# ginolhac/mapDamage

Measured on AMD Instinct MI355X. Metric: reads/sec (misincorporation+comp tables), higher is better.
Workload: dtype u8

## Files before the change

### include/mdx.h

```cpp
#ifndef MDX_H
#define MDX_H

#include <stdint.h>

#ifdef __cplusplus
extern "C" {
#endif

#define MDX_ABI_VERSION 6

#define MDX_OK 0
#define MDX_ERR_ARG (-1)
#define MDX_ERR_HIP (-2)
#define MDX_ERR_STATE (-3)
#define MDX_ERR_MASK_INDEX (-4)
#define MDX_ERR_LGD_OVERFLOW (-5)
#define MDX_ERR_BAD_READ (-6)

#define MDX_ERR_UNSUPPORTED (-8)
#define MDX_ERR_COMM (-7)

#define MDX_FLAG_QUAL_ABOVE_MIN 0x8000
#define MDX_FLAG_HAS_QUAL 0x4000

// ... 145 lines not shown
                       uint8_t *d_qual_out, double *d_mr_raw, uint8_t *d_status);
int mdx_tabulate_rescale_device(mdx_ctx *ctx, const mdx_batch *dev_batch, const int32_t *d_mtid, const int32_t *d_mpos,
                                uint8_t *d_qual_out, double *d_mr_raw, uint8_t *d_status);
int mdx_rescale_patches_device(mdx_ctx *ctx, const mdx_batch *dev_batch, const int32_t *d_mtid, const int32_t *d_mpos,
                               uint64_t *d_patch, int64_t patch_cap, int32_t n_parts, uint64_t *d_n_patch, double *d_mr_raw,
                               uint8_t *d_status);
int mdx_tabulate_rescale_patches_device(mdx_ctx *ctx, const mdx_batch *dev_batch, const int32_t *d_mtid, const int32_t *d_mpos,
                                        uint64_t *d_patch, int64_t patch_cap, int32_t n_parts, uint64_t *d_n_patch, double *d_mr_raw,
                                        uint8_t *d_status);
int mdx_rescale_expand_device(mdx_ctx *ctx, const mdx_batch *dev_batch, const uint64_t *d_patch, int64_t patch_cap, int32_t n_parts,
                              const uint64_t *d_n_patch, uint8_t *d_qual_out);
int mdx_rescale_timing_read(mdx_ctx *ctx, int64_t *n_launches, double *total_ms);
int64_t mdx_fused_launches(const mdx_ctx *ctx);
int64_t mdx_packed_launches(const mdx_ctx *ctx);
int64_t mdx_geo_spec_launches(const mdx_ctx *ctx);
int64_t mdx_libsorts(const mdx_ctx *ctx);
int mdx_last_launch_geometry(const mdx_ctx *ctx, int32_t out[4]);
int64_t mdx_rescale_summary_words(const mdx_ctx *ctx);
int mdx_rescale_summary(mdx_ctx *ctx, uint64_t *words);

typedef struct mdx_source mdx_source;
int mdx_source_open(const char *path, mdx_source **out);
const char *mdx_source_error(const mdx_source *source);
int mdx_source_is_stream(const mdx_source *source);
int mdx_source_peek(mdx_source *source, uint8_t *buf, int32_t n, int32_t *got);
int64_t mdx_source_read(mdx_source *source, uint8_t *buf, int64_t cap);
int mdx_source_seek(mdx_source *source, int64_t offset);
void mdx_source_close(mdx_source *source);

typedef struct mdx_bam mdx_bam;
// ... 141 lines not shown
```

### mapdamage_amd/build.py

```python

import os
import pathlib
import shutil
import subprocess

HERE = pathlib.Path(__file__).resolve().parent
CSRC = HERE / "csrc"
LIB = HERE / "libmdx.so"
SOURCES = ["mdx_kernels.hip", "mdx_rescale.hip", "mdx_capi.cpp", "mdx_bamio.cpp", "mdx_gbam.hip", "mdx_samio.cpp", "mdx_gsam.hip", "mdx_libsort.hip", "mdx_strata.hip", "mdx_fasta.hip", "mdx_stats.hip", "mdx_dedup.hip", "mdx_depth.hip", "mdx_pileup.hip"]
HEADERS = [CSRC / "mdx_internal.h", CSRC / "mdx_filter.h", CSRC / "mdx_damage_key.h", CSRC / "mdx_pmd_key.h", CSRC / "mdx_dup_key.h", CSRC / "mdx_dup_table.h", CSRC / "mdx_depth_key.h", CSRC / "mdx_pileup_key.h", CSRC / "mdx_kept.h", CSRC / "mdx_kept_tags.h", CSRC / "mdx_kept_index.h", CSRC / "mdx_kept_mask.h", CSRC / "mdx_kept_md.h", CSRC / "mdx_device.h", CSRC / "mdx_inflate.h", CSRC / "mdx_deflate.h", CSRC / "mdx_crc32.h", HERE.parent / "include" / "mdx.h"]


def hipcc():
    exe = shutil.which("hipcc") or "/opt/rocm/bin/hipcc"
    if not os.path.exists(exe):
        raise RuntimeError("hipcc not found; the HIP extension cannot be built")
    return exe


def needs_build():
    if not LIB.exists():
        return True
    t = LIB.stat().st_mtime
    deps = [CSRC / s for s in SOURCES] + HEADERS
    return any(p.stat().st_mtime > t for p in deps)
# ... 51 lines not shown
```

### mapdamage_amd/csrc/mdx_capi.cpp

```cpp
#include "../../include/mdx.h"
#include "mdx_internal.h"

#include <dlfcn.h>

#include <chrono>

#include <cstdio>
#include <cstdlib>
#include <cstring>
#include <mutex>
#include <new>
#include <string>
#include <thread>
#include <utility>
#include <vector>

namespace {

constexpr size_t kLdsLimit = MDX_LDS_LIMIT;
#ifdef MDX_WAVE_CLK
static unsigned long long *g_dbg_clk = nullptr;
extern "C" int mdx_dbg_clk_read(unsigned long long *out, int n) {
    if (!g_dbg_clk) return -1;
    (void)hipDeviceSynchronize();
// ... 102 lines not shown
    int st_turn = 0;
    void *gbam_arena = nullptr;
    size_t gbam_arena_cap = 0;
    void *gbam_tables = nullptr;
    void *gbam_stream = nullptr, *gbam_event = nullptr;
    int64_t record_base = 0;
    DevBuf unpacked;
    DevBuf lists;
    DevBuf rs_part;
    DevBuf rs_lists;
    DevBuf rs_in;
    uint32_t *d_tile_ctr = nullptr;
    size_t fuse_prepared = 0;
    size_t pkf_prepared = 0;
    MdxPkConfig pk = {512, 0};
    bool tile_ctr_clean = false;
    bool pkm_prepared = false;
    DevBuf lowq;
    DevBuf libsort;
    DevBuf libsort_scratch;
    const void *libsort_checked = nullptr;
    uint64_t libsort_checked_sig = 0;
    DevBuf ml_partials;
    struct Strata {
        StrataKind kind = STRATA_NONE;
        int n_groups = 0;
        unsigned long long *d_strata_kept = nullptr;
        int32_t *d_group_of_tid = nullptr;
        int strata_n_contig = 0;
        void *d_regions = nullptr;
        MdxRegions regions = {};
// ... 95 lines not shown
    } while (0)

#define HIP_TRY(ctx, call)                                                                     \
    do {                                                                                       \
        hipError_t e_ = (call);                                                                \
        if (e_ != hipSuccess)                                                                  \
            return fail((ctx), MDX_ERR_HIP, std::string(#call) + ": " + hipGetErrorString(e_)); \
    } while (0)

int64_t lgd_words(const mdx_ctx *c) { return (int64_t)c->cfg.nlib * 4 * c->cfg.lgd_max; }
int64_t mis_words(const mdx_ctx *c) { return (int64_t)c->cfg.nlib * 4 * c->cfg.length * MDX_N_MIS_COLS; }
int64_t comp_words(const mdx_ctx *c) { return (int64_t)c->cfg.nlib * 4 * (c->cfg.length + c->cfg.around) * 4; }

size_t pmd_hist_words(const mdx_ctx *c) { return (size_t)(c->cfg.nlib / (c->strata.pmd_n_thresholds + 1)) * MDX_PMD_BINS + 1; }

int zero_accumulators(mdx_ctx *c) {
    HIP_TRY(c, hipMemsetAsync(c->d_raw, 0, (size_t)c->dims.w_total * 8, c->stream));
    HIP_TRY(c, hipMemsetAsync(c->d_lgd_dense, 0, (size_t)lgd_words(c) * 8 * c->lgd_copies, c->stream));
    HIP_TRY(c, hipMemsetAsync(c->d_n_lgd_over, 0, 8, c->stream));
    HIP_TRY(c, hipMemsetAsync(c->d_err, 0xFF, 8, c->stream));
    if (c->strata.d_strata_kept) HIP_TRY(c, hipMemsetAsync(c->strata.d_strata_kept, 0, (size_t)c->cfg.nlib * 8, c->stream));
    if (c->strata.d_pmd_hist) HIP_TRY(c, hipMemsetAsync(c->strata.d_pmd_hist, 0, pmd_hist_words(c) * 8, c->stream));
    return MDX_OK;
}

template <class Key>
Key key_args(const mdx_ctx *c, const mdx_batch *b) {
    Key k{};
    k.n = b->n_reads; k.n_cigar = b->n_cigar; k.n_bases = b->n_bases;
    k.flag = b->flag; k.lib = b->lib; k.tid = b->tid; k.pos = b->pos;
    k.cigar_off = b->cigar_off; k.cigar = b->cigar; k.seq_off = b->seq_off; k.seq = b->seq;
// ... 156 lines not shown
        delete c;
        return MDX_ERR_HIP;
    }
    *out = c;
    if (cfg->nlib > 65535)
        return fail(c, MDX_ERR_ARG, "more than 65535 tables (libraries x reference groups): the 16-bit library column names "
                                    "no more, 0xFFFF being the record without a library");
    HIP_TRY(c, hipSetDevice(cfg->device));
    hipDeviceProp_t prop;
    HIP_TRY(c, hipGetDeviceProperties(&prop, cfg->device));
    c->n_cu = prop.multiProcessorCount > 0 ? prop.multiProcessorCount : 256;
    if (const char *e = getenv("MDX_TEST_CUS")) {
        const int n = atoi(e);
        if (n >= 1 && n < c->n_cu) c->n_cu = n;
    }
    HIP_TRY(c, hipStreamCreateWithFlags(&c->own_stream, hipStreamNonBlocking));
    c->stream = c->own_stream;
    lap("context, stream");

    const int lgd_lds = mdx_k_lgd_lds(cfg->length, cfg->around, cfg->lgd_max);
    if ((int64_t)cfg->nlib * (4LL * cfg->length * 29 + 8LL * (2LL * cfg->around + 512) +
                              4LL * lgd_lds + 128) > 0x7FFFFFF0LL || cfg->length > (1 << 24) || cfg->around > (1 << 24))
        return fail(c, MDX_ERR_ARG, "table too large (nlib * length)");
    c->dims = mdx_make_dims(cfg->length, cfg->around, cfg->nlib, cfg->lgd_max, lgd_lds);
    int group = cfg->nlib;
    while (group > 1 && mdx_k_lds_bytes(mdx_make_dims(cfg->length, cfg->around, group, cfg->lgd_max, lgd_lds)) > kLdsLimit)
        group--;
    const MdxDims gdims = mdx_make_dims(cfg->length, cfg->around, group, cfg->lgd_max, lgd_lds);
    c->lds_bytes = mdx_k_lds_bytes(gdims);
    if (c->lds_bytes <= kLdsLimit) {
        c->mode = MDX_MODE_LDS;
        c->lib_group = group;
        c->max_grid = c->n_cu * (2048 / mdx_k_block_threads());
        HIP_TRY(c, mdx_k_prepare(c->lds_bytes));
        {
            const MdxDims d1 = mdx_make_dims(cfg->length, cfg->around, 1, cfg->lgd_max, lgd_lds);
            c->pk = mdx_k_pk_config(d1, kLdsLimit);
            HIP_TRY(c, mdx_k_prepare_packed(mdx_k_pk_lds_bytes(d1, c->pk)));
            if (const char *e = getenv("MDX_DEBUG_PK")) if (*e && *e != '0')
                fprintf(stderr, "[mdx] packed kernels: blocks of %d threads, %zu bytes of LDS, columns %s\n", c->pk.threads, mdx_k_pk_lds_bytes(d1, c->pk),
                        c->pk.pfl ? "prefetched into the LDS" : "by plain loads");
        }
        lap("kernels");
        HIP_TRY(c, hipMalloc((void **)&c->d_partials, (size_t)c->max_grid * gdims.w_total * 4));
    } else {
        c->mode = MDX_MODE_GLOBAL;
        c->max_grid = c->n_cu * (2048 / mdx_k_block_threads());
    }
    HIP_TRY(c, hipMalloc((void **)&c->d_raw, (size_t)c->dims.w_total * 8));
    c->lgd_copies = mdx_lgd_copies_for(cfg->nlib, cfg->lgd_max);
    HIP_TRY(c, hipMalloc((void **)&c->d_lgd_dense, (size_t)lgd_words(c) * 8 * c->lgd_copies));
    HIP_TRY(c, hipMalloc((void **)&c->d_lgd_over, (size_t)(cfg->lgd_over_cap > 0 ? cfg->lgd_over_cap : 1) * 32));
    HIP_TRY(c, hipMalloc((void **)&c->d_n_lgd_over, 8));
    HIP_TRY(c, hipMalloc((void **)&c->d_err, 8));
    int rc = zero_accumulators(c);
    if (rc != MDX_OK) return rc;
    HIP_TRY(c, hipStreamSynchronize(c->stream));
    lap("accumulators");
    return MDX_OK;
// ... 477 lines not shown
            const int64_t n_tiles = (b->n_reads + T - 1) / T;
            const int64_t n_pools = mdx_n_pools((unsigned)grid);
            const int64_t chunk = MDX_POOL_CHUNK;
            const int64_t pool_tiles = ((n_tiles + n_pools * chunk - 1) / (n_pools * chunk)) * chunk, pool_waves = (grid / n_pools) * wpb_l;
            const bool quota = fuse || (pmask && !ml);
            a.tile_quota = quota ? (int)(2 * ((pool_tiles + pool_waves - 1) / pool_waves) + 2) : 0x7FFFFFFF;
            a.list_cap = fuse ? (int64_t)a.tile_quota * T + 128 : 0;
            a.round_tiles = MDX_ROUND_TILES;
            a.ring_size = MDX_LIST_RING;
            if (quota) while ((int64_t)a.ring_size < (int64_t)a.tile_quota * T + 128) a.ring_size *= 2;
            if (!c->d_tile_ctr) {
                HIP_TRY(c, hipMalloc((void **)&c->d_tile_ctr, (size_t)MDX_CTR_WORDS * 4));
                HIP_TRY(c, hipMemsetAsync(c->d_tile_ctr, 0, (size_t)MDX_CTR_WORDS * 4, c->stream));
            }
            if (n_pools * MDX_CTR_PAD > MDX_CTR_WORDS / 2 || n_pools * MDX_CTR_PAD > MDX_CTR_WORDS) return fail(c, MDX_ERR_STATE, "more blocks than tile counters");
            a.tile_ctr = c->d_tile_ctr;
            {
                const size_t list_bytes = (size_t)nwaves * (size_t)MDX_WAVE_SCRATCH(a.ring_size) * 16;
                if (c->lists.reserve(list_bytes) != hipSuccess)
                    return fail(c, MDX_ERR_HIP, "the per-wavefront lists of this launch (" + std::to_string(list_bytes >> 20) + " MiB) could not be allocated" +
                                (quota ? ": tabulate the batch in smaller pieces" : ""));
            }
            a.lists = (uint4 *)c->lists.p;
            c->last_geom[0] = grid; c->last_geom[1] = wpb_l; c->last_geom[2] = (int32_t)n_tiles; c->last_geom[3] = (int32_t)n_pools;
        }
        hipEvent_t e0 = nullptr, e1 = nullptr;
        if (c->timing) {
            HIP_TRY(c, hipEventCreate(&e0));
            HIP_TRY(c, hipEventCreate(&e1));
            HIP_TRY(c, hipEventRecord(e0, c->stream));
        }
        mdx_batch b_fold;
        const mdx_batch *bs = b;
        if (pmask && !folded) {
            if (lo == 0) {
                HIP_TRY(c, c->lowq.reserve(((size_t)b->n_bases + 1) / 2 + 64));
                const bool bits = b->lowq != nullptr;
                if (b->libsort) return fail(c, MDX_ERR_ARG, "mdx_batch::libsort of a MDX_SEQ_4BIT batch under --min-basequal: upload the batch with the context it is tabulated with");
                mdx_k_fold_mask(b->seq, (uint8_t *)c->lowq.p, b->qual, bits ? b->lowq : nullptr, b->n_bases, c->cfg.minqual, c->stream);
                HIP_TRY(c, hipGetLastError());
// ... 29 lines not shown
                    c->n_libsorts++;
                }
                blob = c->libsort.p;
            }
            MdxLibSort ls;
            mdx_k_libsort_layout(const_cast<void *>(blob), b->n_reads, b->n_cigar, b->n_bases, c->cfg.nlib, &ls);
            if (c->strata.n_groups > 0 && b->libsort && lo == 0) mdx_k_strata_kept_from_sort(ls.lib_start, c->cfg.nlib, c->strata.d_strata_kept, c->stream);
            a.flag = ls.flag; a.tid = ls.tid; a.pos = ls.pos; a.tlen = ls.tlen;
            a.cigar_off = ls.cigar_off; a.cigar = ls.cigar; a.seq_off = ls.seq_off; a.seq = ls.seq;
            a.perm = ls.perm; a.lib_start = ls.lib_start; a.sort_bad = ls.bad;
            HIP_TRY(c, c->ml_partials.reserve((size_t)mdx_n_pools((unsigned)grid) * 16));
            a.ml_plan = (const uint4 *)c->ml_partials.p;
            mdx_k_ml_plan(ls.lib_start, lo, gn, mdx_tile_records(a.dims, a.pfl_off != 0), grid, c->ml_partials.p, c->stream);
        }
        const size_t n_ctr = (size_t)mdx_n_pools((unsigned)grid);
        if (!c->tile_ctr_clean || n_ctr > 4096) HIP_TRY(c, hipMemsetAsync(c->d_tile_ctr, 0, n_ctr * MDX_CTR_PAD * 4, c->stream));
        c->tile_ctr_clean = false;
        if (fuse) {
            HIP_TRY(c, hipMemsetAsync(fuse->mr_raw, 0xFF, (size_t)b->n_reads * 8, c->stream));
            const int64_t nwaves = (int64_t)grid * wpb_l;
            HIP_TRY(c, c->rs_in.reserve((size_t)nwaves * (size_t)(a.list_cap + 1) * 4));
            a.rs.gen_count = (uint32_t *)c->rs_in.p;
            a.rs.gen_list = a.rs.gen_count + nwaves;
            if (packed) { mdx_k_tabulate_packed_fused(a, grid, lds, c->stream); c->n_packed++; }
            else mdx_k_tabulate_fused(a, grid, lds, c->stream);
            c->fuse_list_cap = a.list_cap;
            if (fused_grid) *fused_grid = grid;
        } else if (packed) {
            if (pmask) mdx_k_tabulate_packed_masked(a, grid, c->pk.threads, lds, c->stream);
            else if (mdx_k_tabulate_packed(a, grid, c->pk.threads, lds, c->stream)) c->n_geo_spec++;
            c->n_packed++;
        } else {
            mdx_k_tabulate(a, c->mode, mask, grid, lds, c->stream);
        }
        if (c->timing) {
            HIP_TRY(c, hipEventRecord(e1, c->stream));
            c->events.emplace_back(e0, e1);
        }
        HIP_TRY(c, hipGetLastError());
        if (c->mode == MDX_MODE_LDS) {
            if (ml) mdx_k_reduce_partials(c->d_partials, a.raw, c->d_raw + c->dims.w_total - 1, a.dims.w_total, grid, c->stream, c->d_tile_ctr, gn, c->dims.w_lib, a.ml_plan);
            else
            mdx_k_reduce_partials(c->d_partials, a.raw, c->d_raw + c->dims.w_total - 1, a.dims.w_total, grid, c->stream, c->d_tile_ctr);
            c->tile_ctr_clean = a.dims.w_total >= 4096 && n_ctr <= 4096;
            HIP_TRY(c, hipGetLastError());
        }
    }
    return MDX_OK;
}

int mdx_tabulate_device(mdx_ctx *c, const mdx_batch *b) { return tabulate_impl(c, b, nullptr, nullptr); }

int mdx_tabulate_host(mdx_ctx *c, const mdx_batch *h) {
    int rc = check_batch(c, h);
    if (rc != MDX_OK) return rc;
    if (h->n_reads == 0) return MDX_OK;
    HIP_TRY(c, hipSetDevice(c->cfg.device));
    const int64_t n = h->n_reads;
    const void *src[10] = {h->flag, h->lib, h->tid, h->pos, h->tlen, h->cigar_off, h->cigar, h->seq_off, h->seq, h->qual};
// ... 73 lines not shown
        std::snprintf(msg, sizeof msg, "record %lld (index within its batch + the record base): %s", (long long)(err >> 8), mdx_strerror(code));
        return fail(c, code, msg);
    }
    if ((int64_t)nover > c->cfg.lgd_over_cap) return fail(c, MDX_ERR_LGD_OVERFLOW, mdx_strerror(MDX_ERR_LGD_OVERFLOW));
    return MDX_OK;
}

int64_t mdx_table_words(const mdx_ctx *c) {
    if (!c) return 0;
    return mis_words(c) + comp_words(c) + lgd_words(c) + 2;
}

int mdx_finish_device(mdx_ctx *c, uint64_t *d_tables) {
    if (!c || !d_tables) return MDX_ERR_ARG;
    HIP_TRY(c, hipSetDevice(c->cfg.device));
    mdx_k_finalize(c->d_raw, c->d_lgd_dense, c->d_n_lgd_over, c->dims, c->lgd_copies, (unsigned long long *)d_tables, c->stream);
    HIP_TRY(c, hipGetLastError());
    return MDX_OK;
}

int mdx_comm_unique_id(uint8_t *id) {
    if (!id) return MDX_ERR_ARG;
    const Rccl *r = rccl();
    if (!r) return MDX_ERR_COMM;
    RcclId u;
    if (r->GetUniqueId(&u) != 0) return MDX_ERR_COMM;
    std::memcpy(id, u.internal, MDX_COMM_ID_BYTES);
    return MDX_OK;
}

// ... 1236 lines not shown
    if (e == hipSuccess) e = hipStreamSynchronize(c->stream);
    if (e == hipSuccess) e = hipMemcpy(qual_out, d_qout, (size_t)h->n_bases, hipMemcpyDeviceToHost);
    if (e == hipSuccess) e = hipMemcpy(mr_raw, d_mr, (size_t)n * 8, hipMemcpyDeviceToHost);
    if (e == hipSuccess) e = hipMemcpy(status, d_status, (size_t)n, hipMemcpyDeviceToHost);
    void *tmp[] = {d_mtid, d_mpos, d_qout, d_status, d_mr};
    for (void *p : tmp) if (p) (void)hipFree(p);
    (void)mdx_batch_free(c, &dv);
    if (rc != MDX_OK) return rc;
    if (e != hipSuccess) return fail(c, MDX_ERR_HIP, hipGetErrorString(e));
    return mdx_sync(c, nullptr);
}

int64_t mdx_fused_launches(const mdx_ctx *c) { return c ? c->n_fused : -1; }
int64_t mdx_packed_launches(const mdx_ctx *c) { return c ? c->n_packed : -1; }
int64_t mdx_geo_spec_launches(const mdx_ctx *c) { return c ? c->n_geo_spec : -1; }
int64_t mdx_libsorts(const mdx_ctx *c) { return c ? c->n_libsorts : -1; }
int mdx_last_launch_geometry(const mdx_ctx *c, int32_t out[4]) {
    if (!c || !out) return MDX_ERR_ARG;
    for (int i = 0; i < 4; i++) out[i] = c->last_geom[i];
    return MDX_OK;
}

int mdx_rescale_timing_read(mdx_ctx *c, int64_t *n_launches, double *total_ms) {
    if (!c) return MDX_ERR_ARG;
    HIP_TRY(c, hipStreamSynchronize(c->stream));
    double tot = 0;
    int64_t n = 0;
    for (auto &ev : c->rs_events) {
        float ms = 0;
        if (hipEventElapsedTime(&ms, ev.first, ev.second) == hipSuccess) { tot += ms; n++; }
// ... 30 lines not shown
```

### mapdamage_amd/csrc/mdx_internal.h

```cpp
#pragma once

#include <hip/hip_runtime.h>
#include <stdint.h>

#include <string>
#include <vector>

struct MdxDims {
    int L, A, nlib, lgd_max, lgd_lds;
    int nl8;
    int G, R;
    int nl16, G4, H4;
    int t_pad;
    int w_mis, w_cmp, w_mc, w_tc, w_dmp, w_lgd, w_lib;
    int64_t w_total;
    __host__ __device__ int off_tc() const { return 0; }
    __host__ __device__ int off_mis() const { return w_tc; }
    __host__ __device__ int off_cmp() const { return w_tc + w_mis; }
    __host__ __device__ int off_dmp() const { return w_tc + w_mc; }
    __host__ __device__ int off_lgd() const { return w_tc + w_mc + w_dmp; }
    __host__ __device__ int tau_left(int p) const { const int b = p + A; return 64 * (b & 7) + (b >> 3); }
    __host__ __device__ int tau_right(int p) const { const int e = p + A; return 64 * (7 - (e & 7)) + nl8 + (e >> 3); }
    __host__ __device__ int tau_lflank(int dist) const {
        if (nl8 == 0) return dist - 1;
// ... 7 lines not shown
    }
    __host__ __device__ bool fast_ok() const { return nl8 > 0; }
};

#define MDX_MAX_R 4
#ifndef MDX_POOL_BLOCKS
#define MDX_POOL_BLOCKS 2
#endif
static inline __host__ __device__ unsigned mdx_n_pools(unsigned grid) {
    return (grid >= MDX_POOL_BLOCKS && grid % MDX_POOL_BLOCKS == 0u) ? grid / MDX_POOL_BLOCKS : ((grid >= 2u && !(grid & 1u)) ? grid / 2u : grid);
}
#ifndef MDX_CTR_PAD
#define MDX_CTR_PAD 32
#endif
#define MDX_CTR_WORDS 262144
#define MDX_ML_MAX_LIBS 64
#ifndef MDX_POOL_CHUNK
#define MDX_POOL_CHUNK 24
#endif
static constexpr inline __host__ __device__ int mdx_stage_entries(const MdxDims &d) {
    return d.R > 0 ? 64 - 64 % d.R + d.R - 1 : 64;
}
#define MDX_LGD_COPIES 32
#define MDX_LGD_COPIES_BYTES ((int64_t)1 << 30)
static inline int mdx_lgd_copies_for(int nlib, int lgd_max) {
    int copies = MDX_LGD_COPIES;
    while (copies > 1 && (int64_t)copies * nlib * 4 * lgd_max * 8 > MDX_LGD_COPIES_BYTES) copies >>= 1;
    return copies;
}

// ... 55 lines not shown
    const int32_t *tlen;
    const uint32_t *cigar_off;
    const uint32_t *cigar;
    const uint32_t *seq_off;
    const uint8_t *seq;
    const uint8_t *qual;
    const uint8_t *ref;
    const uint8_t *ref4;
    int ref2;
    int seq_packed;
    const int64_t *contig_off;
    int n_contig;
    int minqual;
    MdxDims dims;
    uint32_t *partials;
    unsigned long long *raw;
    unsigned long long *lgd_dense;
    int lgd_copies;
    long long *lgd_over;
    long long lgd_over_cap;
    unsigned long long *n_lgd_over;
    unsigned long long *err;
    long long record_base;
    int stage_off;
    int queue_off;
    int pfl_off;
    int ref32;
    int64_t n_bases;
    int lib_lo, nlib_total;
    uint4 *lists;
    int ring_size;
    int64_t list_cap;
    MdxFuse rs;
    uint32_t *tile_ctr;
    const uint4 *ml_plan;
    int tile_quota;
    int round_tiles;
    const uint32_t *perm, *lib_start;
    const unsigned long long *sort_bad;
    int n_libs;
#ifdef MDX_WAVE_CLK
    unsigned long long *dbg_clk;
#endif
};
#ifndef MDX_PK_QCAP
#define MDX_PK_QCAP 112
#endif

enum { MDX_MODE_LDS = 0, MDX_MODE_GLOBAL = 1 };
// ... 369 lines not shown
```

### mapdamage_amd/csrc/mdx_kernels.hip

```cpp
#include "mdx_device.h"

#include <type_traits>

typedef u32x4 __attribute__((aligned(16))) u32x4_a;
__device__ __forceinline__ void cp_store(u8 *p, const u32x4 v) { *(u32x4_a *)p = v; }
__device__ __forceinline__ u32x4 cp_load(const u8 *p) { return *(const u32x4_a *)p; }
__device__ __forceinline__ u32x3 ld12_stream(const u8 *p) { return *(const u32x3 *)p; }

#ifndef MDX_BLOCK
#define MDX_BLOCK 768
#endif
#ifndef MDX_WPS
#define MDX_WPS 6
#endif
#ifndef PIPE_DEPTH
#define PIPE_DEPTH 4
#endif
#ifndef MDX_PD_G
#define MDX_PD_G 2
#endif
#ifndef MDX_PD_P
#define MDX_PD_P 3
#endif
#ifndef MDX_PK_PD
// ... 461 lines not shown
    constexpr bool pfl = PFLC;
    extern __shared__ __attribute__((aligned(16))) u32 lds[];
    constexpr MdxDims geo_d = MdxGeo::dims;
    MdxDims d_ = GEOC ? geo_d : a.dims;
    if (GEOC) d_.lgd_max = a.dims.lgd_max;
    const MdxDims d = d_;
    const int L = d.L, A = d.A;
    const int k_stage_off = GEOC ? MdxGeo::stage_off : a.stage_off, k_queue_off = GEOC ? MdxGeo::queue_off : a.queue_off,
              k_pfl_off = GEOC ? MdxGeo::pfl_off : a.pfl_off, k_lib_lo = GEOC ? 0 : a.lib_lo;
    const int lane = threadIdx.x & 63;
    const int wave = __builtin_amdgcn_readfirstlane((int)(threadIdx.x >> 6));
    const int waves_per_block = BLOCK / 64;
    const u32 gwave = blockIdx.x * waves_per_block + wave;
    const u32 nwaves = gridDim.x * waves_per_block;
    u64 *raw = a.raw;
#ifdef MDX_WAVE_CLK
    if (a.dbg_clk && lane == 0) a.dbg_clk[3 * (size_t)gwave] = wall_clock64();
#endif
#ifdef MDX_PHASE_CLK
    u32 ph_acc[16] = {0u, 0u, 0u, 0u, 0u, 0u, 0u, 0u, 0u, 0u, 0u, 0u, 0u, 0u, 0u, 0u};
    int ph_cur = 0;
    u64 ph_t0 = __builtin_amdgcn_s_memtime();
#define MDX_PH(id) do { const u64 t_ = __builtin_amdgcn_s_memtime(); const u32 dt_ = (u32)__builtin_amdgcn_readfirstlane((int)(u32)(t_ - ph_t0)); \
        _Pragma("unroll") for (int q_ = 0; q_ < 16; q_++) ph_acc[q_] += ph_cur == q_ ? dt_ : 0u; ph_t0 = t_; ph_cur = (id); } while (0)
#define MDX_PH_IN(id) const int ph_prev_ = ph_cur; MDX_PH(id)
#define MDX_PH_OUT() MDX_PH(ph_prev_)
#define MDX_PH_IMPL(x) x##_impl
#else
#define MDX_PH_IMPL(x) x
#define MDX_PH(id) do { } while (0)
// ... 2047 lines not shown
            int v4[4] = {tA + bcA, tC + bcC, tG + bcG, tT + bcT};
            for (int b = 0; b < 4; b++) {
                int v = v4[b];
                for (int o = 32; o; o >>= 1) v += __shfl_xor(v, o);
                if (lane == 0 && v) atomicAdd(&rs_cnt[b], (u32)v);
            }
            __syncthreads();
            for (int i = threadIdx.x; i < n_tcb; i += BLOCK) {
                const int lib = i / d.w_tc, j = i - lib * d.w_tc;
                lds[lib * d.w_lib + d.off_tc() + j] += lds[a.rs.tcb_off + i];
            }
            if (threadIdx.x < 4) a.rs.subs_part[(size_t)blockIdx.x * rs_ncnt + threadIdx.x] = rs_cnt[threadIdx.x];
            __syncthreads();
        }
        u32 *out = a.partials + (i64)blockIdx.x * d.w_total;
        if (PK) {
            for (int i = threadIdx.x; i < d.w_tc; i += BLOCK) {
                const int w = i & 511, k = (i >> 9) & 3, strand = (i >> 11) & 1;
                const int ln = w & 63, jb = w >> 6;
                u32 v = 0u;
                if (ln < d.G) {
                    const int side = ln >= d.nl8, m = ln - side * d.nl8;
                    const int wn = side ? 8 * m + 7 - jb : 8 * m + jb;
                    if (wn < A + L) {
                        const int j = side ? 15 - (wn & 15) : (wn & 15);
                        for (int gs = 0; gs < d.H4; gs++)
                            v += lds[d.off_tc() + (k << 10) + 64 * j + (strand * d.H4 + gs) * d.G4 + side * d.nl16 + (wn >> 4)];
                    }
                }
                out[d.off_tc() + i] = v;
            }
            for (i64 i = d.w_tc + threadIdx.x; i < d.w_total; i += BLOCK) out[i] = lds[i];
        } else
        for (i64 i = threadIdx.x; i < d.w_total; i += BLOCK) out[i] = lds[i];
    }
    }
}

template <bool MASK, bool FAST>
static hipError_t prep_one(size_t lds_bytes) {
    return hipFuncSetAttribute((const void *)tabulate_kernel<true, MASK, FAST>,
                               hipFuncAttributeMaxDynamicSharedMemorySize, (int)lds_bytes);
}

hipError_t mdx_k_fuse_prepare(size_t lds_bytes) {
    return hipFuncSetAttribute((const void *)tabulate_kernel<true, false, true, true>,
                               hipFuncAttributeMaxDynamicSharedMemorySize, (int)lds_bytes);
}

// ... 361 lines not shown
```

### mapdamage_amd/engine.py

```python

import ctypes
import os
import pathlib

import numpy as np

from . import layout as L
from .batch import ReadBatch, Reference
from .tables import TableSet

_HERE = pathlib.Path(__file__).resolve().parent
_LIBPATH = _HERE / "libmdx.so"
_lib = None

EXPORTS = (
    "mdx_abi_version", "mdx_strerror", "mdx_create", "mdx_destroy", "mdx_last_error",
    "mdx_set_stream", "mdx_set_reference", "mdx_batch_upload", "mdx_batch_free",
    "mdx_tabulate_host", "mdx_tabulate_device", "mdx_sync", "mdx_table_words",
    "mdx_finish_device", "mdx_finish", "mdx_reset", "mdx_timing_enable", "mdx_timing_read",
    "mdx_table_mode", "mdx_genome_composition", "mdx_rescale_set_model", "mdx_rescale_host",
    "mdx_rescale_summary_words", "mdx_rescale_summary",
    "mdx_comm_unique_id", "mdx_comm_init", "mdx_comm_adopt", "mdx_comm_size", "mdx_finish_allreduce",
    "mdx_rescale_device", "mdx_tabulate_rescale_device", "mdx_rescale_timing_read", "mdx_fused_launches",
    "mdx_bam_read", "mdx_bam_free", "mdx_bam_error", "mdx_bam_header_text", "mdx_bam_n_ref", "mdx_bam_ref_name",
# ... 4 lines not shown
    "mdx_gbam_at_end", "mdx_gbam_close", "mdx_gbam_set_min_basequal", "mdx_gbam_missing_qualities",
    "mdx_gbam_inflate_blocks", "mdx_set_record_base", "mdx_pack_seq", "mdx_gbam_set_seq_format", "mdx_packed_launches", "mdx_geo_spec_launches",
    "mdx_gbam_skip", "mdx_comm_count", "mdx_gbam_tell", "mdx_gbam_fixups", "mdx_bam_seek", "mdx_libsorts",
    "mdx_gbam_view_flags", "mdx_gbam_view_set_flags",
    "mdx_rescale_patches_device", "mdx_tabulate_rescale_patches_device", "mdx_rescale_expand_device", "mdx_mr_round", "mdx_batch_fold", "mdx_bgzf_deflate",
    "mdx_gbam_rescale_slab", "mdx_gbam_write_rescaled", "mdx_gbam_record_name", "mdx_gbam_kept_bound", "mdx_gbam_write_kept",
    "mdx_gbam_kept_bound_tagged", "mdx_gbam_write_kept_tagged", "mdx_gbam_kept_index", "mdx_gbam_kept_index_linear", "mdx_gbam_set_kept_mask", "mdx_gbam_kept_mask_counts",
    "mdx_gbam_set_kept_md", "mdx_gbam_kept_md_counts", "mdx_gbam_kept_bound_md", "mdx_strata_pmd_keep_scores", "mdx_strata_pmd_scores",
    "mdx_fasta_index", "mdx_set_reference_fasta", "mdx_fasta_load_stats", "mdx_reference_fetch", "mdx_host_threads", "mdx_host_pool_threads", "mdx_warm",
    "mdx_source_open", "mdx_source_error", "mdx_source_is_stream", "mdx_source_peek", "mdx_source_read", "mdx_source_close",
    "mdx_bam_read_source", "mdx_bam_open_source", "mdx_gbam_open_source",
    "mdx_source_seek", "mdx_gsam_open", "mdx_gsam_open_source", "mdx_gsam_header", "mdx_gsam_error", "mdx_gsam_configure",
    "mdx_gsam_set_seq_format", "mdx_gsam_set_min_basequal", "mdx_gsam_next", "mdx_gsam_at_end", "mdx_gsam_tell",
    "mdx_gsam_view_flags", "mdx_gsam_view_set_flags", "mdx_gsam_missing_qualities", "mdx_gsam_close",
    "mdx_gsam_is_bgzf", "mdx_gsam_tell_bgzf",
    "mdx_last_launch_geometry",
    "mdx_set_strata", "mdx_set_strata_regions", "mdx_set_strata_damage", "mdx_set_strata_pmd", "mdx_strata_pmd_histogram", "mdx_strata_pmd_unqualified", "mdx_strata_groups", "mdx_strata_kept", "mdx_merged_words", "mdx_finish_merged", "mdx_finish_merged_host", "mdx_lgd_copies",
    "mdx_stats_loglik", "mdx_stats_run", "mdx_stats_pmat",
    "mdx_bam_apply_record_filter", "mdx_gbam_set_record_filter", "mdx_gbam_filter_counts", "mdx_gsam_set_record_filter",
    "mdx_gsam_filter_counts",
    "mdx_dedup_begin", "mdx_dedup_mark", "mdx_dedup_counts", "mdx_dedup_histogram", "mdx_dedup_info",
    "mdx_depth_begin", "mdx_depth_add", "mdx_depth_finish", "mdx_depth_runs", "mdx_depth_fetch", "mdx_depth_info", "mdx_depth_regions",
    "mdx_pileup_begin", "mdx_pileup_add", "mdx_pileup_finish", "mdx_pileup_info",
)

SEQ_ASCII, SEQ_4BIT, SEQ_4BITQ = 0, 1, 2


class MdxPileupConfig(ctypes.Structure):
    _fields_ = [("min_basequal", ctypes.c_int32), ("mask5", ctypes.c_int32), ("mask3", ctypes.c_int32), ("call", ctypes.c_int32),
                ("min_depth", ctypes.c_int32), ("single_strand", ctypes.c_int32), ("seed", ctypes.c_uint64)]
# ... 59 lines not shown
    lib.mdx_comm_size.argtypes = [ctypes.c_void_p]
    lib.mdx_comm_count.argtypes = [ctypes.c_void_p]
    lib.mdx_comm_adopt.argtypes = [ctypes.c_void_p, ctypes.c_void_p, ctypes.c_int32, ctypes.c_int32]
    lib.mdx_rescale_summary_words.restype = ctypes.c_int64
    lib.mdx_rescale_summary_words.argtypes = [ctypes.c_void_p]
    lib.mdx_fused_launches.restype = ctypes.c_int64
    lib.mdx_fused_launches.argtypes = [ctypes.c_void_p]
    lib.mdx_packed_launches.restype = ctypes.c_int64
    lib.mdx_packed_launches.argtypes = [ctypes.c_void_p]
    lib.mdx_geo_spec_launches.restype = ctypes.c_int64
    lib.mdx_geo_spec_launches.argtypes = [ctypes.c_void_p]
    lib.mdx_libsorts.restype = ctypes.c_int64
    lib.mdx_libsorts.argtypes = [ctypes.c_void_p]
    lib.mdx_last_launch_geometry.restype = ctypes.c_int
    lib.mdx_last_launch_geometry.argtypes = [ctypes.c_void_p, ctypes.c_void_p]
    for name in ("mdx_bam_error", "mdx_bam_header_text", "mdx_bam_ref_name", "mdx_bam_rg_name"):
        getattr(lib, name).restype = ctypes.c_char_p
    lib.mdx_bam_qnames.restype = ctypes.c_void_p
    lib.mdx_bam_qmin.restype = ctypes.c_void_p
    lib.mdx_bam_qmin.argtypes = [ctypes.c_void_p]
    lib.mdx_bam_ref_length.restype = ctypes.c_int64
    lib.mdx_bam_free.restype = None
    for name in ("mdx_bam_error", "mdx_bam_header_text", "mdx_bam_n_ref", "mdx_bam_n_rg", "mdx_bam_free"):
        getattr(lib, name).argtypes = [ctypes.c_void_p]
    for name in ("mdx_bam_ref_name", "mdx_bam_ref_length", "mdx_bam_rg_name"):
        getattr(lib, name).argtypes = [ctypes.c_void_p, ctypes.c_int32]
    lib.mdx_bam_stream_header.restype = ctypes.c_void_p
    lib.mdx_bam_stream_header.argtypes = [ctypes.c_void_p]
    lib.mdx_bam_next.argtypes = [ctypes.c_void_p, ctypes.c_int64, ctypes.c_void_p]
    lib.mdx_bam_close.restype = None
# ... 595 lines not shown
    def rescale_expand(self, dbatch, d_patch, patch_cap, n_parts, d_n_patch, d_qual_out):
        dev = dbatch.dev if isinstance(dbatch, DeviceBatch) else dbatch
        self._lib.mdx_rescale_expand_device.restype = ctypes.c_int
        self._check(self._lib.mdx_rescale_expand_device(self._ctx, ctypes.byref(dev), ctypes.c_void_p(d_patch), ctypes.c_int64(patch_cap),
                                                        ctypes.c_int32(n_parts), ctypes.c_void_p(d_n_patch), ctypes.c_void_p(d_qual_out)))

    def fused_launches(self):
        return int(self._lib.mdx_fused_launches(self._ctx))

    def packed_launches(self):
        return int(self._lib.mdx_packed_launches(self._ctx))

    def geo_spec_launches(self):
        return int(self._lib.mdx_geo_spec_launches(self._ctx))

    def libsorts(self):
        return int(self._lib.mdx_libsorts(self._ctx))

    def last_launch_geometry(self):
        out = np.zeros(4, np.int32)
        self._check(self._lib.mdx_last_launch_geometry(self._ctx, _ptr(out)))
        return dict(zip(("grid", "waves_per_block", "tiles", "pools"), (int(x) for x in out)))

    def rescale_timing_read(self):
        n = ctypes.c_int64(0)
        ms = ctypes.c_double(0)
        self._check(self._lib.mdx_rescale_timing_read(self._ctx, ctypes.byref(n), ctypes.byref(ms)))
        return n.value, ms.value

    def rescale_summary(self):
# ... 17 lines not shown
```

Before: 27.50 billion.

## Defer per-block partials reduction across batches with accumulating partial slots

```diff
diff --git a/include/mdx.h b/include/mdx.h
--- a/include/mdx.h
+++ b/include/mdx.h
@@ -183,6 +183,7 @@
 int64_t mdx_fused_launches(const mdx_ctx *ctx);
 int64_t mdx_packed_launches(const mdx_ctx *ctx);
 int64_t mdx_geo_spec_launches(const mdx_ctx *ctx);
+int mdx_partials_info(const mdx_ctx *ctx, int64_t out[4]);
 int64_t mdx_libsorts(const mdx_ctx *ctx);
 int mdx_last_launch_geometry(const mdx_ctx *ctx, int32_t out[4]);
 int64_t mdx_rescale_summary_words(const mdx_ctx *ctx);
diff --git a/mapdamage_amd/build.py b/mapdamage_amd/build.py
--- a/mapdamage_amd/build.py
+++ b/mapdamage_amd/build.py
@@ -8,7 +8,7 @@
 CSRC = HERE / "csrc"
 LIB = HERE / "libmdx.so"
 SOURCES = ["mdx_kernels.hip", "mdx_rescale.hip", "mdx_capi.cpp", "mdx_bamio.cpp", "mdx_gbam.hip", "mdx_samio.cpp", "mdx_gsam.hip", "mdx_libsort.hip", "mdx_strata.hip", "mdx_fasta.hip", "mdx_stats.hip", "mdx_dedup.hip", "mdx_depth.hip", "mdx_pileup.hip"]
-HEADERS = [CSRC / "mdx_internal.h", CSRC / "mdx_filter.h", CSRC / "mdx_damage_key.h", CSRC / "mdx_pmd_key.h", CSRC / "mdx_dup_key.h", CSRC / "mdx_dup_table.h", CSRC / "mdx_depth_key.h", CSRC / "mdx_pileup_key.h", CSRC / "mdx_kept.h", CSRC / "mdx_kept_tags.h", CSRC / "mdx_kept_index.h", CSRC / "mdx_kept_mask.h", CSRC / "mdx_kept_md.h", CSRC / "mdx_device.h", CSRC / "mdx_inflate.h", CSRC / "mdx_deflate.h", CSRC / "mdx_crc32.h", HERE.parent / "include" / "mdx.h"]
+HEADERS = [CSRC / "mdx_internal.h", CSRC / "mdx_partials.h", CSRC / "mdx_filter.h", CSRC / "mdx_damage_key.h", CSRC / "mdx_pmd_key.h", CSRC / "mdx_dup_key.h", CSRC / "mdx_dup_table.h", CSRC / "mdx_depth_key.h", CSRC / "mdx_pileup_key.h", CSRC / "mdx_kept.h", CSRC / "mdx_kept_tags.h", CSRC / "mdx_kept_index.h", CSRC / "mdx_kept_mask.h", CSRC / "mdx_kept_md.h", CSRC / "mdx_device.h", CSRC / "mdx_inflate.h", CSRC / "mdx_deflate.h", CSRC / "mdx_crc32.h", HERE.parent / "include" / "mdx.h"]
 
 
 def hipcc():
diff --git a/mapdamage_amd/csrc/mdx_capi.cpp b/mapdamage_amd/csrc/mdx_capi.cpp
--- a/mapdamage_amd/csrc/mdx_capi.cpp
+++ b/mapdamage_amd/csrc/mdx_capi.cpp
@@ -1,5 +1,6 @@
 #include "../../include/mdx.h"
 #include "mdx_internal.h"
+#include "mdx_partials.h"
 
 #include <dlfcn.h>
 
@@ -140,7 +141,19 @@
     size_t fuse_prepared = 0;
     size_t pkf_prepared = 0;
     MdxPkConfig pk = {512, 0};
-    bool tile_ctr_clean = false;
+    bool tile_ctr_clean[2] = {false, false};
+    struct LazyPartials {
+        bool eager = false;
+        int64_t limit = MDX_PARTIALS_MAX_RECORDS;
+        bool pending = false;
+        int grid = 0;
+        int64_t records = 0;
+        unsigned long long *raw = nullptr;
+        int64_t w_total = 0;
+        size_t stale_words = 0;
+        uint64_t n_lazy = 0;
+        int64_t n_flushes = 0, n_eager = 0;
+    } lazy;
     bool pkm_prepared = false;
     DevBuf lowq;
     DevBuf libsort;
@@ -266,7 +279,26 @@
 
 size_t pmd_hist_words(const mdx_ctx *c) { return (size_t)(c->cfg.nlib / (c->strata.pmd_n_thresholds + 1)) * MDX_PMD_BINS + 1; }
 
+int zero_partial_slots(mdx_ctx *c) {
+    mdx_ctx::LazyPartials &z = c->lazy;
+    const size_t pending_words = z.pending ? (size_t)z.grid * (size_t)z.w_total : 0;
+    const size_t words = pending_words > z.stale_words ? pending_words : z.stale_words;
+    if (words) HIP_TRY(c, hipMemsetAsync(c->d_partials, 0, words * 4, c->stream));
+    z.pending = false; z.grid = 0; z.records = 0; z.raw = nullptr; z.w_total = 0; z.stale_words = 0;
+    return MDX_OK;
+}
+
+int flush_partials(mdx_ctx *c) {
+    mdx_ctx::LazyPartials &z = c->lazy;
+    if (!z.pending) return MDX_OK;
+    mdx_k_reduce_partials(c->d_partials, z.raw, z.raw + z.w_total - 1, z.w_total, z.grid, c->stream);
+    HIP_TRY(c, hipGetLastError());
+    z.n_flushes++;
+    return zero_partial_slots(c);
+}
+
 int zero_accumulators(mdx_ctx *c) {
+    if (c->d_partials) { int rc = zero_partial_slots(c); if (rc != MDX_OK) return rc; }
     HIP_TRY(c, hipMemsetAsync(c->d_raw, 0, (size_t)c->dims.w_total * 8, c->stream));
     HIP_TRY(c, hipMemsetAsync(c->d_lgd_dense, 0, (size_t)lgd_words(c) * 8 * c->lgd_copies, c->stream));
     HIP_TRY(c, hipMemsetAsync(c->d_n_lgd_over, 0, 8, c->stream));
@@ -453,6 +485,8 @@
         const int n = atoi(e);
         if (n >= 1 && n < c->n_cu) c->n_cu = n;
     }
+    if (const char *e = getenv("MDX_EAGER_PARTIALS")) c->lazy.eager = *e && *e != '0';
+    if (const char *e = getenv("MDX_PARTIALS_FLUSH_READS")) c->lazy.limit = mdx_partials_limit(atoll(e));
     HIP_TRY(c, hipStreamCreateWithFlags(&c->own_stream, hipStreamNonBlocking));
     c->stream = c->own_stream;
     lap("context, stream");
@@ -482,6 +516,7 @@
         }
         lap("kernels");
         HIP_TRY(c, hipMalloc((void **)&c->d_partials, (size_t)c->max_grid * gdims.w_total * 4));
+        HIP_TRY(c, hipMemsetAsync(c->d_partials, 0, (size_t)c->max_grid * gdims.w_total * 4, c->stream));
     } else {
         c->mode = MDX_MODE_GLOBAL;
         c->max_grid = c->n_cu * (2048 / mdx_k_block_threads());
@@ -989,7 +1024,6 @@
                 HIP_TRY(c, hipMemsetAsync(c->d_tile_ctr, 0, (size_t)MDX_CTR_WORDS * 4, c->stream));
             }
             if (n_pools * MDX_CTR_PAD > MDX_CTR_WORDS / 2 || n_pools * MDX_CTR_PAD > MDX_CTR_WORDS) return fail(c, MDX_ERR_STATE, "more blocks than tile counters");
-            a.tile_ctr = c->d_tile_ctr;
             {
                 const size_t list_bytes = (size_t)nwaves * (size_t)MDX_WAVE_SCRATCH(a.ring_size) * 16;
                 if (c->lists.reserve(list_bytes) != hipSuccess)
@@ -999,6 +1033,17 @@
             a.lists = (uint4 *)c->lists.p;
             c->last_geom[0] = grid; c->last_geom[1] = wpb_l; c->last_geom[2] = (int32_t)n_tiles; c->last_geom[3] = (int32_t)n_pools;
         }
+        mdx_ctx::LazyPartials &z = c->lazy;
+        const bool lazy = !z.eager && c->mode == MDX_MODE_LDS && !ml && !fuse && c->cfg.nlib == 1 && a.raw == c->d_raw;
+        if (c->mode == MDX_MODE_LDS) {
+            if (z.pending && (!lazy || z.raw != a.raw || z.w_total != a.dims.w_total || mdx_partials_must_flush(z.records, b->n_reads, z.limit)) &&
+                (rc = flush_partials(c)) != MDX_OK) return rc;
+            if (lazy && z.stale_words && (rc = zero_partial_slots(c)) != MDX_OK) return rc;
+        }
+        a.partials_accumulate = lazy ? 1 : 0;
+        const int ctr_set = lazy ? (int)(z.n_lazy & 1) : 0;
+        a.tile_ctr = c->d_tile_ctr + (size_t)ctr_set * MDX_CTR_SET_LINES * MDX_CTR_PAD;
+        a.tile_ctr_zero = lazy ? c->d_tile_ctr + (size_t)(ctr_set ^ 1) * MDX_CTR_SET_LINES * MDX_CTR_PAD : nullptr;
         hipEvent_t e0 = nullptr, e1 = nullptr;
         if (c->timing) {
             HIP_TRY(c, hipEventCreate(&e0));
@@ -1058,8 +1103,8 @@
             mdx_k_ml_plan(ls.lib_start, lo, gn, mdx_tile_records(a.dims, a.pfl_off != 0), grid, c->ml_partials.p, c->stream);
         }
         const size_t n_ctr = (size_t)mdx_n_pools((unsigned)grid);
-        if (!c->tile_ctr_clean || n_ctr > 4096) HIP_TRY(c, hipMemsetAsync(c->d_tile_ctr, 0, n_ctr * MDX_CTR_PAD * 4, c->stream));
-        c->tile_ctr_clean = false;
+        if (!c->tile_ctr_clean[ctr_set] || n_ctr > 4096) HIP_TRY(c, hipMemsetAsync(a.tile_ctr, 0, n_ctr * MDX_CTR_PAD * 4, c->stream));
+        c->tile_ctr_clean[ctr_set] = false;
         if (fuse) {
             HIP_TRY(c, hipMemsetAsync(fuse->mr_raw, 0xFF, (size_t)b->n_reads * 8, c->stream));
             const int64_t nwaves = (int64_t)grid * wpb_l;
@@ -1082,11 +1127,21 @@
             c->events.emplace_back(e0, e1);
         }
         HIP_TRY(c, hipGetLastError());
-        if (c->mode == MDX_MODE_LDS) {
+        if (lazy) {
+            z.pending = true;
+            if (grid > z.grid) z.grid = grid;
+            z.records += b->n_reads;
+            z.raw = a.raw; z.w_total = a.dims.w_total;
+            z.n_lazy++;
+            c->tile_ctr_clean[ctr_set ^ 1] = true;
+        } else if (c->mode == MDX_MODE_LDS) {
+            const size_t stored = (size_t)grid * (size_t)a.dims.w_total;
+            if (stored > z.stale_words) z.stale_words = stored;
+            z.n_eager++;
             if (ml) mdx_k_reduce_partials(c->d_partials, a.raw, c->d_raw + c->dims.w_total - 1, a.dims.w_total, grid, c->stream, c->d_tile_ctr, gn, c->dims.w_lib, a.ml_plan);
             else
             mdx_k_reduce_partials(c->d_partials, a.raw, c->d_raw + c->dims.w_total - 1, a.dims.w_total, grid, c->stream, c->d_tile_ctr);
-            c->tile_ctr_clean = a.dims.w_total >= 4096 && n_ctr <= 4096;
+            c->tile_ctr_clean[0] = a.dims.w_total >= 4096 && n_ctr <= 4096;
             HIP_TRY(c, hipGetLastError());
         }
     }
@@ -1190,6 +1245,8 @@
 int mdx_finish_device(mdx_ctx *c, uint64_t *d_tables) {
     if (!c || !d_tables) return MDX_ERR_ARG;
     HIP_TRY(c, hipSetDevice(c->cfg.device));
+    int rc = flush_partials(c);
+    if (rc != MDX_OK) return rc;
     mdx_k_finalize(c->d_raw, c->d_lgd_dense, c->d_n_lgd_over, c->dims, c->lgd_copies, (unsigned long long *)d_tables, c->stream);
     HIP_TRY(c, hipGetLastError());
     return MDX_OK;
@@ -2456,6 +2513,11 @@
 int64_t mdx_fused_launches(const mdx_ctx *c) { return c ? c->n_fused : -1; }
 int64_t mdx_packed_launches(const mdx_ctx *c) { return c ? c->n_packed : -1; }
 int64_t mdx_geo_spec_launches(const mdx_ctx *c) { return c ? c->n_geo_spec : -1; }
+int mdx_partials_info(const mdx_ctx *c, int64_t out[4]) {
+    if (!c || !out) return MDX_ERR_ARG;
+    out[0] = (int64_t)c->lazy.n_lazy; out[1] = c->lazy.n_flushes; out[2] = c->lazy.n_eager; out[3] = c->lazy.pending ? c->lazy.records : 0;
+    return MDX_OK;
+}
 int64_t mdx_libsorts(const mdx_ctx *c) { return c ? c->n_libsorts : -1; }
 int mdx_last_launch_geometry(const mdx_ctx *c, int32_t out[4]) {
     if (!c || !out) return MDX_ERR_ARG;
diff --git a/mapdamage_amd/csrc/mdx_internal.h b/mapdamage_amd/csrc/mdx_internal.h
--- a/mapdamage_amd/csrc/mdx_internal.h
+++ b/mapdamage_amd/csrc/mdx_internal.h
@@ -45,6 +45,7 @@
 #define MDX_CTR_PAD 32
 #endif
 #define MDX_CTR_WORDS 262144
+#define MDX_CTR_SET_LINES (MDX_CTR_WORDS / 2 / MDX_CTR_PAD)
 #define MDX_ML_MAX_LIBS 64
 #ifndef MDX_POOL_CHUNK
 #define MDX_POOL_CHUNK 24
@@ -130,6 +131,7 @@
     int minqual;
     MdxDims dims;
     uint32_t *partials;
+    int partials_accumulate;
     unsigned long long *raw;
     unsigned long long *lgd_dense;
     int lgd_copies;
@@ -149,6 +151,7 @@
     int64_t list_cap;
     MdxFuse rs;
     uint32_t *tile_ctr;
+    uint32_t *tile_ctr_zero;
     const uint4 *ml_plan;
     int tile_quota;
     int round_tiles;
diff --git a/mapdamage_amd/csrc/mdx_kernels.hip b/mapdamage_amd/csrc/mdx_kernels.hip
--- a/mapdamage_amd/csrc/mdx_kernels.hip
+++ b/mapdamage_amd/csrc/mdx_kernels.hip
@@ -499,6 +499,8 @@
     const u32 gwave = blockIdx.x * waves_per_block + wave;
     const u32 nwaves = gridDim.x * waves_per_block;
     u64 *raw = a.raw;
+    if (a.tile_ctr_zero)
+        for (u32 i = blockIdx.x * (u32)BLOCK + threadIdx.x; i < (u32)MDX_CTR_SET_LINES; i += gridDim.x * (u32)BLOCK) a.tile_ctr_zero[i * MDX_CTR_PAD] = 0u;
 #ifdef MDX_WAVE_CLK
     if (a.dbg_clk && lane == 0) a.dbg_clk[3 * (size_t)gwave] = wall_clock64();
 #endif
@@ -2576,6 +2578,7 @@
             __syncthreads();
         }
         u32 *out = a.partials + (i64)blockIdx.x * d.w_total;
+        const bool acc = a.partials_accumulate != 0;
         if (PK) {
             for (int i = threadIdx.x; i < d.w_tc; i += BLOCK) {
                 const int w = i & 511, k = (i >> 9) & 3, strand = (i >> 11) & 1;
@@ -2590,11 +2593,12 @@
                             v += lds[d.off_tc() + (k << 10) + 64 * j + (strand * d.H4 + gs) * d.G4 + side * d.nl16 + (wn >> 4)];
                     }
                 }
+                if (acc) v += out[d.off_tc() + i];
                 out[d.off_tc() + i] = v;
             }
-            for (i64 i = d.w_tc + threadIdx.x; i < d.w_total; i += BLOCK) out[i] = lds[i];
+            for (i64 i = d.w_tc + threadIdx.x; i < d.w_total; i += BLOCK) out[i] = acc ? out[i] + lds[i] : lds[i];
         } else
-        for (i64 i = threadIdx.x; i < d.w_total; i += BLOCK) out[i] = lds[i];
+        for (i64 i = threadIdx.x; i < d.w_total; i += BLOCK) out[i] = acc ? out[i] + lds[i] : lds[i];
     }
     }
 }
diff --git a/mapdamage_amd/csrc/mdx_partials.h b/mapdamage_amd/csrc/mdx_partials.h
--- /dev/null
+++ b/mapdamage_amd/csrc/mdx_partials.h
@@ -0,0 +1,12 @@
+#pragma once
+#include <cstdint>
+
+constexpr int64_t MDX_PARTIALS_MAX_RECORDS = 0x7FFFFFFFLL;
+
+constexpr int64_t mdx_partials_limit(int64_t wanted) {
+    return wanted >= 1 && wanted < MDX_PARTIALS_MAX_RECORDS ? wanted : MDX_PARTIALS_MAX_RECORDS;
+}
+
+constexpr bool mdx_partials_must_flush(int64_t pending, int64_t next, int64_t limit = MDX_PARTIALS_MAX_RECORDS) {
+    return pending > 0 && next > mdx_partials_limit(limit) - pending;
+}
diff --git a/mapdamage_amd/engine.py b/mapdamage_amd/engine.py
--- a/mapdamage_amd/engine.py
+++ b/mapdamage_amd/engine.py
@@ -42,7 +42,7 @@
     "mdx_gsam_set_seq_format", "mdx_gsam_set_min_basequal", "mdx_gsam_next", "mdx_gsam_at_end", "mdx_gsam_tell",
     "mdx_gsam_view_flags", "mdx_gsam_view_set_flags", "mdx_gsam_missing_qualities", "mdx_gsam_close",
     "mdx_gsam_is_bgzf", "mdx_gsam_tell_bgzf",
-    "mdx_last_launch_geometry",
+    "mdx_last_launch_geometry", "mdx_partials_info",
     "mdx_set_strata", "mdx_set_strata_regions", "mdx_set_strata_damage", "mdx_set_strata_pmd", "mdx_strata_pmd_histogram", "mdx_strata_pmd_unqualified", "mdx_strata_groups", "mdx_strata_kept", "mdx_merged_words", "mdx_finish_merged", "mdx_finish_merged_host", "mdx_lgd_copies",
     "mdx_stats_loglik", "mdx_stats_run", "mdx_stats_pmat",
     "mdx_bam_apply_record_filter", "mdx_gbam_set_record_filter", "mdx_gbam_filter_counts", "mdx_gsam_set_record_filter",
@@ -132,6 +132,9 @@
     lib.mdx_libsorts.argtypes = [ctypes.c_void_p]
     lib.mdx_last_launch_geometry.restype = ctypes.c_int
     lib.mdx_last_launch_geometry.argtypes = [ctypes.c_void_p, ctypes.c_void_p]
+    if hasattr(lib, "mdx_partials_info"):
+        lib.mdx_partials_info.restype = ctypes.c_int
+        lib.mdx_partials_info.argtypes = [ctypes.c_void_p, ctypes.c_void_p]
     for name in ("mdx_bam_error", "mdx_bam_header_text", "mdx_bam_ref_name", "mdx_bam_rg_name"):
         getattr(lib, name).restype = ctypes.c_char_p
     lib.mdx_bam_qnames.restype = ctypes.c_void_p
@@ -757,6 +760,11 @@
     def geo_spec_launches(self):
         return int(self._lib.mdx_geo_spec_launches(self._ctx))
 
+    def partials_info(self):
+        out = np.zeros(4, np.int64)
+        self._check(self._lib.mdx_partials_info(self._ctx, _ptr(out)))
+        return dict(zip(("lazy_launches", "flushes", "eager_launches", "pending_records"), (int(x) for x in out)))
+
     def libsorts(self):
         return int(self._lib.mdx_libsorts(self._ctx))
 
```

Result: no change. 27.48 billion (median of 2 runs) (-0.1%).
